# xiaozhah/Aligner

Measured on AMD Instinct MI355X. Metric: aligned utterances/sec + frames/sec, [B=64,T_text=200,T_mel=1000], higher is better.
Workload: dtype f32; 1 GPU; configs[1]: similarity (L2, C=80) + monotonic alignment search, [B=64,T_text=200,T_mel=1000] fp32 per GPU, dense fp32 path + int32 durations out; batch_per_gpu=64, t_text=200, t_mel=1000, c_att=80, launch=hipGraph, batches_in_flight=3, parallelism=batch-sharded x1

## Files before the change

aligner_amd/csrc/api.cpp:

```cpp
#include <cstdarg>
#include <cstdio>
#include <cstdlib>

#include <mutex>
#include <cstring>
#include <map>
#include <utility>

#include "common.h"

namespace aligner {

char *error_buffer() {
    static thread_local char buf[512] = {0};
    return buf;
}

unsigned long long *g_debug_stamps = nullptr;

static int env_flag(const char *name) { const char *e = getenv(name); return e && e[0] && e[0] != '0'; }
int g_opt_fwdsum_one_wave = env_flag("ALIGNER_FWDSUM_ONE_WAVE");
int g_opt_fwdsum_serial = env_flag("ALIGNER_FWDSUM_SERIAL");
int g_opt_fwdsum_no_grad_stager = 0;
int g_opt_softattn_exact = env_flag("ALIGNER_SOFTATTN_EXACT");
int g_opt_mobo_drop_segment = -1;
int g_opt_mobo_start_lag = 0;
int g_opt_mobo_lanes = 0;
int g_opt_mobo_bwd_general = 0;
int g_opt_softattn_no_pair = 0;
int g_opt_softattn_rt_drop_merge = 0;
int g_opt_softattn_strips = env_flag("ALIGNER_SOFTATTN_STRIPS");
int g_opt_softattn_split = 0;
int g_opt_conv_narrow_ft = 0;
int g_opt_conv_no_ring = 0;
int g_opt_conv_no_fuse = 0;
int g_opt_conv_split_always = env_flag("ALIGNER_CONV_SPLIT_ALWAYS");
int g_opt_maxpath_no_split_walk = 0;
int g_opt_maxpath_zero_blocks = 0;
int g_opt_maxpath_no_mask_verify = 0;
int g_opt_maxpath_no_optimistic_mask = 0;
int g_opt_mobo_full_chain = 0;
int g_opt_mobo_stamp_wave = 0;

hipError_t ensure_dynamic_lds(const void *kernel, size_t bytes) {
    if (bytes <= 64 * 1024) return hipSuccess;
    int dev = 0;
    hipError_t e = hipGetDevice(&dev);
    if (e != hipSuccess) return e;
    static std::mutex mu;
    static std::map<std::pair<int, const void *>, size_t> granted;
    std::lock_guard<std::mutex> lock(mu);
    const auto key = std::make_pair(dev, kernel);
    auto it = granted.find(key);
    if (it != granted.end() && it->second >= bytes) return hipSuccess;
    e = hipFuncSetAttribute(kernel, hipFuncAttributeMaxDynamicSharedMemorySize, (int)bytes);
    if (e == hipSuccess) granted[key] = bytes;
    return e;
}

int device_cu_count() {
    int dev = 0, v = 0;
    if (hipGetDevice(&dev) != hipSuccess) return 1;
    static std::mutex mu;
    static std::map<int, int> counts;
    std::lock_guard<std::mutex> lock(mu);
    auto it = counts.find(dev);
    if (it != counts.end()) return it->second;
    if (hipDeviceGetAttribute(&v, hipDeviceAttributeMultiprocessorCount, dev) != hipSuccess || v < 1) v = 1;
    counts[dev] = v;
    return v;
}

int device_lds_limit() {
    int dev = 0;
    if (hipGetDevice(&dev) != hipSuccess) return 64 * 1024;
    static std::mutex mu;
    static std::map<int, int> limits;
    std::lock_guard<std::mutex> lock(mu);
    auto it = limits.find(dev);
    if (it != limits.end()) return it->second;
    int lim = 64 * 1024, v = 0;
    hipDeviceProp_t prop;
    if (hipGetDeviceProperties(&prop, dev) == hipSuccess && std::strncmp(prop.gcnArchName, "gfx950", 6) == 0)
        lim = 160 * 1024;
    else if (hipDeviceGetAttribute(&v, hipDeviceAttributeMaxSharedMemoryPerBlock, dev) == hipSuccess && v > 0)
        lim = v;
    limits[dev] = lim;
    return lim;
}

int fail(int code, const char *fmt, ...) {
    va_list ap;
    va_start(ap, fmt);
    vsnprintf(error_buffer(), 512, fmt, ap);
    va_end(ap);
    return code;
}

}

extern "C" {

int aligner_abi_version(void) { return ALIGNER_ABI_VERSION; }

const char *aligner_last_error(void) { return aligner::error_buffer(); }

void aligner_debug_set_stamps(void *stamps_dev) {
    aligner::g_debug_stamps = static_cast<unsigned long long *>(stamps_dev);
}

int aligner_debug_set_option(const char *name, int value) {
    if (!name) return aligner::fail(ALIGNER_EINVAL, "null option name");
    if (std::strcmp(name, "fwdsum_one_wave") == 0) { aligner::g_opt_fwdsum_one_wave = value; return ALIGNER_OK; }
    if (std::strcmp(name, "fwdsum_no_grad_stager") == 0) { aligner::g_opt_fwdsum_no_grad_stager = value; return ALIGNER_OK; }
    if (std::strcmp(name, "fwdsum_serial") == 0) { aligner::g_opt_fwdsum_serial = value; return ALIGNER_OK; }
    if (std::strcmp(name, "softattn_exact") == 0) { aligner::g_opt_softattn_exact = value; return ALIGNER_OK; }
    if (std::strcmp(name, "mobo_start_lag") == 0) { aligner::g_opt_mobo_start_lag = value; return ALIGNER_OK; }
    if (std::strcmp(name, "mobo_lanes") == 0) { aligner::g_opt_mobo_lanes = value; return ALIGNER_OK; }
    if (std::strcmp(name, "mobo_stamp_wave") == 0) { aligner::g_opt_mobo_stamp_wave = value; return ALIGNER_OK; }
    if (std::strcmp(name, "mobo_full_chain") == 0) { aligner::g_opt_mobo_full_chain = value; return ALIGNER_OK; }
    if (std::strcmp(name, "softattn_split") == 0) { aligner::g_opt_softattn_split = value; return ALIGNER_OK; }
    if (std::strcmp(name, "conv_narrow_ft") == 0) { aligner::g_opt_conv_narrow_ft = value; return ALIGNER_OK; }
    if (std::strcmp(name, "conv_no_ring") == 0) { aligner::g_opt_conv_no_ring = value; return ALIGNER_OK; }
    if (std::strcmp(name, "conv_no_fuse") == 0) { aligner::g_opt_conv_no_fuse = value; return ALIGNER_OK; }
    if (std::strcmp(name, "conv_split_always") == 0) { aligner::g_opt_conv_split_always = value; return ALIGNER_OK; }
    if (std::strcmp(name, "maxpath_no_optimistic_mask") == 0) { aligner::g_opt_maxpath_no_optimistic_mask = value; return ALIGNER_OK; }
    if (std::strcmp(name, "maxpath_no_mask_verify") == 0) { aligner::g_opt_maxpath_no_mask_verify = value; return ALIGNER_OK; }
    if (std::strcmp(name, "maxpath_zero_blocks") == 0) { aligner::g_opt_maxpath_zero_blocks = value; return ALIGNER_OK; }
    if (std::strcmp(name, "maxpath_no_split_walk") == 0) { aligner::g_opt_maxpath_no_split_walk = value; return ALIGNER_OK; }
    if (std::strcmp(name, "softattn_strips") == 0) { aligner::g_opt_softattn_strips = value; return ALIGNER_OK; }
    if (std::strcmp(name, "softattn_rt_drop_merge") == 0) { aligner::g_opt_softattn_rt_drop_merge = value; return ALIGNER_OK; }
    if (std::strcmp(name, "softattn_no_pair") == 0) { aligner::g_opt_softattn_no_pair = value; return ALIGNER_OK; }
    if (std::strcmp(name, "mobo_bwd_general") == 0) { aligner::g_opt_mobo_bwd_general = value; return ALIGNER_OK; }
    if (std::strcmp(name, "mobo_drop_segment") == 0) { aligner::g_opt_mobo_drop_segment = value; return ALIGNER_OK; }
    return aligner::fail(ALIGNER_EINVAL, "unknown option '%s'", name);
}

int aligner_device_count(void) {
    int n = 0;
    if (hipGetDeviceCount(&n) != hipSuccess) {
        (void)hipGetLastError();
        return 0;
    }
    return n;
}

}
```

aligner_amd/csrc/common.h:

```cpp
#pragma once
#include <hip/hip_runtime.h>
#include <cstdarg>
#include <cstdio>

#include "aligner_amd.h"

namespace aligner {

char *error_buffer();
int   fail(int code, const char *fmt, ...) __attribute__((format(printf, 2, 3)));

#define ALIGNER_HIP_CHECK(expr)                                                        \
    do {                                                                               \
        hipError_t _e = (expr);                                                        \
        if (_e != hipSuccess)                                                          \
            return ::aligner::fail(ALIGNER_EHIP, "%s failed: %s (%s:%d)", #expr,       \
                                   hipGetErrorString(_e), __FILE__, __LINE__);         \
    } while (0)

inline int dtype_size(int dt) {
    switch (dt) {
        case ALIGNER_DT_F32: return 4;
        case ALIGNER_DT_F16: return 2;
        case ALIGNER_DT_BF16: return 2;
        case ALIGNER_DT_F64: return 8;
        case ALIGNER_DT_I32: return 4;
        case ALIGNER_DT_U8: return 1;
        case ALIGNER_DT_I64: return 8;
        default: return 0;
    }
}

hipError_t ensure_dynamic_lds(const void *kernel, size_t bytes);

int device_lds_limit();
int device_cu_count();

extern unsigned long long *g_debug_stamps;
extern int g_opt_softattn_exact;
extern int g_opt_mobo_start_lag;
extern int g_opt_mobo_stamp_wave;
extern int g_opt_mobo_full_chain;
extern int g_opt_conv_narrow_ft;
extern int g_opt_conv_no_ring;
extern int g_opt_maxpath_no_optimistic_mask;
extern int g_opt_maxpath_no_mask_verify;
extern int g_opt_maxpath_zero_blocks;
extern int g_opt_maxpath_no_split_walk;
extern int g_opt_conv_no_fuse;
extern int g_opt_conv_split_always;
extern int g_opt_softattn_split;
extern int g_opt_softattn_strips;
extern int g_opt_softattn_rt_drop_merge;
extern int g_opt_softattn_no_pair;
extern int g_opt_mobo_bwd_general;
extern int g_opt_mobo_lanes;
extern int g_opt_mobo_drop_segment;
extern int g_opt_fwdsum_no_grad_stager;
extern int g_opt_fwdsum_serial;
extern int g_opt_fwdsum_one_wave;

inline size_t align_up(size_t v, size_t a) { return (v + a - 1) / a * a; }

}
```

aligner_amd/csrc/mobo.hip:

```cpp
#include <hip/hip_runtime.h>

#include <cmath>
#include <cstdint>

#include "aligner_amd.h"
#include "common.h"

namespace aligner {

constexpr float MB_NEG = -1e30f;
constexpr float MB_DEADF = -1e7f;
constexpr int MB_DEADM = -(1 << 24);
constexpr unsigned MB_FILL = 0xFFFFFFFFu;
constexpr float MB_LOG2E = 1.4426950408889634f, MB_LN2 = 0.6931471805599453f;
constexpr int MB_SPIN_LIMIT = 1 << 21;

struct MoboParams {
    const void *e;
    const int *t_xs, *t_ys;
    float *log_alpha;
    int *boundaries;
    int *durations;
    float *map_score;
    float *Lw;
// ... 942 lines not shown
                const unsigned h_c = h_nx;
                issue_halo(i + 1 < I ? i + 1 : I - 1);
                const int bo = (i & 1) * W;
                auto halo_entry = [&](int h, unsigned x) {
                    if (x == MB_FILL) {
                        const unsigned *r = ring_in + (size_t)i * 3 * D + h;
                        int spins = 0;
                        do {
                            __builtin_amdgcn_s_sleep(2);
                            x = mb_ring_load(r);
                            if (++spins > p.spin_limit) gave_up = true;
                        } while (x == MB_FILL && !gave_up);
                    }
                    sV[bo + h] = (x == MB_FILL) ? MB_NEG : __builtin_bit_cast(float, x);
                };
                if (fetches) halo_entry(hl, h_c);
                if (D > 64) {
#pragma unroll 1
                    for (int h = hl + 64; h < D; h += 64) halo_entry(h, MB_FILL);
                }
                mb_lds_barrier();
            }
        }
        if (gave_up) {
            atomicOr(p.status, ALIGNER_ST_INTERNAL);
            p.failw[b] = 1;
        }
        return;
    }

    const int je = (j1 < 1 ? 1 : (j1 > J ? J : j1)) - 1;
    const int kl = j1 > J - 1 ? J - 1 : j1;
    unsigned e_n1, e_n2;
    float L_n1, L_n2;
    auto issue = [&](int i, unsigned &e_o, float &L_o) {
        const size_t ro = ubase + (size_t)i * p.Ty;
        e_o = mb_load_raw<VT>(p.e, ro + je);
        L_o = p.Lw[ro + kl];
    };
    issue(i0, e_n1, L_n1);
    mb_ring_store(trash, 0u);
    mb_ring_store(trash, 0u);
    issue(i0 + 1 < I ? i0 + 1 : I - 1, e_n2, L_n2);
    mb_ring_store(trash, 0u);
    mb_ring_store(trash, 0u);
    auto do_row = [&](const int i, unsigned &e_s, float &L_s) {
        int lo, hi;
        mb_bounds(I, J, D, i, lo, hi);
        const unsigned e_c = e_s;
        const float L_c = L_s;
        issue(i + 2 < I ? i + 2 : I - 1, e_s, L_s);
        const int bo = (i & 1) * W;
        {
            const float L = (j1 < J) ? L_c : MB_NEG;
            float v = (L > MB_DEADF && de > MB_DEADF) ? de - L : MB_NEG;
            v = (v > MB_DEADF) ? v : MB_NEG;
            *(mine ? sV + bo + D + pi : sSpare) = v;
            mb_ring_store(publishes ? ring_out + (size_t)i * 3 * D + (j1 - (bnd - D)) : trash, __builtin_bit_cast(unsigned, v));
        }
        mb_lds_barrier();
        {
            const float ev = mb_value<VT>(e_c) * MB_LOG2E;
            const bool feasible = mine && j1 >= lo && j1 <= hi;
            const float *vv = sV + bo + (mine ? pi : 0) + w0;
            const int cnt = w1 - w0;
            float best = MB_NEG;
            int qb = 0, c = 0;
            for (const int r8 = cnt & 7; c < r8; ++c) {
                const float v = vv[c];
                if (v >= best) { best = v; qb = c; }
            }
#define MB_MAX3F(a_, b_, c_) __builtin_fmaxf(__builtin_fmaxf(a_, b_), c_)
#define MB_MAX3I(a_, b_, c_) ((a_) > (b_) ? ((a_) > (c_) ? (a_) : (c_)) : ((b_) > (c_) ? (b_) : (c_)))
            if (((cnt - c) & 15) == 0) {
#pragma unroll 1
                for (; c < cnt; c += 16) {
                    float v[16];
#pragma unroll
                    for (int u = 0; u < 16; ++u) v[u] = vv[c + u];
                    const float m0 = MB_MAX3F(v[0], v[1], v[2]), m1 = MB_MAX3F(v[3], v[4], v[5]), m2 = MB_MAX3F(v[6], v[7], v[8]);
                    const float m3 = MB_MAX3F(v[9], v[10], v[11]), m4 = MB_MAX3F(v[12], v[13], v[14]);
                    const float vm = __builtin_fmaxf(MB_MAX3F(m0, m1, m2), MB_MAX3F(m3, m4, v[15]));
                    int q[16];
#pragma unroll
                    for (int u = 0; u < 16; ++u) q[u] = (v[u] == vm) ? u : -1;
                    const int q0 = MB_MAX3I(q[0], q[1], q[2]), q1 = MB_MAX3I(q[3], q[4], q[5]), q2 = MB_MAX3I(q[6], q[7], q[8]);
                    const int q3 = MB_MAX3I(q[9], q[10], q[11]), q4 = MB_MAX3I(q[12], q[13], q[14]);
                    const int qa = MB_MAX3I(q0, q1, q2), qc = MB_MAX3I(q3, q4, q[15]);
                    const int qi = qa > qc ? qa : qc;
                    const bool take = vm >= best;
                    best = take ? vm : best;
                    qb = take ? c + qi : qb;
                }
            } else {
#pragma unroll 1
                for (; c < cnt; c += 8) {
                    float v[8];
#pragma unroll
                    for (int u = 0; u < 8; ++u) v[u] = vv[c + u];
                    float vm = v[0];
#pragma unroll
                    for (int u = 1; u < 8; ++u) vm = __builtin_fmaxf(vm, v[u]);
                    int qi = 0;
#pragma unroll
                    for (int u = 1; u < 8; ++u) qi = (v[u] == vm) ? u : qi;
                    if (vm >= best) { best = vm; qb = c + qi; }
                }
            }
#undef MB_MAX3F
#undef MB_MAX3I
            qb += w0;
#pragma unroll
            for (int m = 1; m < H; m <<= 1) {
                const float bo_ = mb_quad_xor_f(best, m);
                const int qo = mb_quad_xor_i(qb, m);
                const bool take = bo_ > best || (bo_ == best && qo > qb);
                best = take ? bo_ : best;
                qb = take ? qo : qb;
            }
            float dev = MB_NEG;
            int dur = 0;
            if (feasible && ev > MB_DEADF && best > MB_DEADF) {
                dev = ev + best;
                dur = D - qb;
                if (!(dev > MB_DEADF)) { dev = MB_NEG; dur = 0; }
            }
            de = dev;
            unsigned short *bp = lead ? backb + (size_t)i * p.bstride + j1 : reinterpret_cast<unsigned short *>(trash);
            *bp = (unsigned short)dur;
        }
    };
#pragma unroll 1
    for (int i = i0; i <= i1; i += 2) {
        do_row(i, e_n1, L_n1);
        if (i + 1 > i1) break;
        do_row(i + 1, e_n2, L_n2);
    }
    if (lead && j1 == J && i1 == I - 1 && p.map_score)
        p.map_score[b] = (de > MB_DEADF) ? de * MB_LN2 : -__builtin_huge_valf();
    if (i1 + 1 < I) {
        const int i = i1 + 1;
        if (publishes) {
            const float Lr = p.Lw[ubase + (size_t)i * p.Ty + kl];
            const float L = (j1 < J) ? Lr : MB_NEG;
            float v = (L > MB_DEADF && de > MB_DEADF) ? de - L : MB_NEG;
            v = (v > MB_DEADF) ? v : MB_NEG;
            mb_ring_store(ring_out + (size_t)i * 3 * D + (j1 - (bnd - D)), __builtin_bit_cast(unsigned, v));
        }
        dead_rows(i1 + 2, I);
        if (lead && j1 == J && p.map_score) p.map_score[b] = -__builtin_huge_valf();
    }
}

template <int VT, int H>
__global__ __launch_bounds__(1024) void mobo_chain_sum_kernel(MoboParams p) {
    extern __shared__ __attribute__((aligned(16))) unsigned char smem[];
    const int tid = threadIdx.x;
    const bool has_helper = p.S > 1;
    const int T = (int)blockDim.x - (has_helper ? 64 : 0);
    const bool helper = tid >= T;
    const int b = blockIdx.x / p.S, sg = blockIdx.x - b * p.S;
    const int D = p.D;
    int I = p.t_xs[b], J = p.t_ys[b];
    I = I > p.Tx ? p.Tx : I;
    J = J > p.Ty ? p.Ty : J;
    const bool ok = I >= 1 && J >= I && (long long)J <= (long long)I * D;
    if (!ok) {
        if (sg == 0 && tid == 0) atomicOr(p.status, ALIGNER_ST_BAD_LENGTHS);
        return;
    }
    const int P = J + 1;
    int Sb = P / D;
    Sb = Sb < 1 ? 1 : (Sb > p.S ? p.S : Sb);
    const int n = (P + Sb - 1) / Sb;
    const int a = sg * n;
    if (sg >= Sb || a >= P) return;
    const int bnd = (a + n < P) ? a + n : P;
    const bool has_next = (sg + 1 < Sb) && (a + n < P) && sg != p.drop_seg;
    const int W = p.nmax + D;
    int *sM = reinterpret_cast<int *>(smem);
    float *sS = reinterpret_cast<float *>(sM + 2 * W);
    float *sT = sS + 2 * W;
    int *sRep = reinterpret_cast<int *>(sT + 2 * W);
    float *sSpare = reinterpret_cast<float *>(sRep + 64);
    if (tid < 32) { sRep[2 * tid] = MB_DEADM; sRep[2 * tid + 1] = 0; }
    for (int h = tid; h < D; h += T) {
        sM[h] = MB_DEADM;  sM[W + h] = MB_DEADM;
        sS[h] = 0.f;       sS[W + h] = 0.f;
        sT[h] = 0.f;       sT[W + h] = 0.f;
    }
    mb_lds_barrier();
    const int pi = tid / H, sub = tid - pi * H;
    const int j1 = a + pi;
    const bool mine = !helper && j1 < bnd;
    const bool lead = mine && sub == 0;
    float la = (j1 == 0) ? 0.f : MB_NEG;
    const size_t ubase = (size_t)b * p.Tx * p.Ty;
    unsigned *trash = p.trash + (size_t)blockIdx.x * 1024 + tid;
    unsigned *ring_out = p.ring + ((size_t)b * (p.S - 1) + (has_next ? sg : 0)) * (size_t)p.Tx * 3 * D;
    const unsigned *ring_in = p.ring + ((size_t)b * (p.S - 1) + (sg > 0 ? sg - 1 : 0)) * (size_t)p.Tx * 3 * D;
    const int hl = tid - T;
    const bool publishes = has_next && lead && j1 >= bnd - D;
    const int w0 = (sub * D) / H, w1 = ((sub + 1) * D) / H;
    const int wave = tid >> 6, lane = tid & 63;
    int i0, i1;
    mb_active_rows(I, J, D, a, bnd, i0, i1);
    auto dead_rows = [&](int from, int to) {
        for (int i = from; i < to; ++i) {
            if (has_next && !helper)
                for (int h = tid; h < D; h += T) {
                    unsigned *r = ring_out + (size_t)i * 3 * D + h;
                    mb_ring_store(r, __builtin_bit_cast(unsigned, (float)MB_DEADM));
                    mb_ring_store(r + D, 0u);
                }
            if (lead && j1 >= 1) p.log_alpha[ubase + (size_t)i * p.Ty + (j1 - 1)] = -__builtin_huge_valf();
        }
    };
    if (i1 < 0) {
        dead_rows(0, I);
        return;
    }
    dead_rows(0, i0);
    bool gave_up = false;
    int R = 0;

    if (helper) {
        if (sg > 0) {
            if (p.start_lag > 0) {
                int ig = i0 + p.start_lag;
                ig = ig > I - 1 ? I - 1 : ig;
                const unsigned *r = ring_in + (size_t)ig * 3 * D + (hl < D ? hl : 0) + D;
                int spins = 0;
                while (mb_ring_load(r) == MB_FILL && !gave_up) {
                    __builtin_amdgcn_s_sleep(8);
                    if (++spins > p.spin_limit) gave_up = true;
                }
            }
            const bool fetches = hl < D;
            unsigned h0_nx, h1_nx;
            auto issue_halo = [&](int i) {
                const unsigned *r = fetches ? ring_in + (size_t)i * 3 * D + hl : trash;
                h0_nx = mb_ring_load(r);
                h1_nx = mb_ring_load(r + (fetches ? D : 0));
            };
            issue_halo(i0);
#pragma unroll 1
            for (int i = i0; i <= i1; ++i) {
                const unsigned h_c0 = h0_nx, h_c1 = h1_nx;
                issue_halo(i + 1 < I ? i + 1 : I - 1);
                const int bo = (i & 1) * W;
                int Mstat = MB_DEADM;
                bool fits = true;
                auto halo_entry = [&](int h, unsigned x0, unsigned x1) {
                    if (x0 == MB_FILL || x1 == MB_FILL) {
                        const unsigned *r = ring_in + (size_t)i * 3 * D + h;
                        int spins = 0;
                        do {
                            __builtin_amdgcn_s_sleep(2);
                            x0 = mb_ring_load(r);
                            x1 = mb_ring_load(r + D);
                            if (++spins > p.spin_limit) gave_up = true;
                        } while ((x0 == MB_FILL || x1 == MB_FILL) && !gave_up);
                    }
                    const bool bad = (x0 == MB_FILL || x1 == MB_FILL);
                    const int M = bad ? MB_DEADM : (int)__builtin_bit_cast(float, x0);
                    const float sv = bad ? 0.f : __builtin_bit_cast(float, x1);
                    sM[bo + h] = M;
                    sS[bo + h] = sv;
                    sT[bo + h] = __builtin_ldexpf(sv, M - R);
                    if (M != MB_DEADM) {
                        Mstat = Mstat > M ? Mstat : M;
                        fits = fits && M >= R - 100 && M <= R + 100;
                    }
                };
                if (fetches) halo_entry(hl, h_c0, h_c1);
                if (D > 64) {
#pragma unroll 1
                    for (int h = hl + 64; h < D; h += 64) halo_entry(h, MB_FILL, MB_FILL);
                }
                {
                    const int wm = mb_wave_max_i32(Mstat);
                    const bool wfit = __builtin_amdgcn_ballot_w64(!fits) == 0;
                    mb_report_put(sRep, i & 1, wave, wm, wfit ? 0 : 1);
                }
                mb_lds_barrier();
                int Rn, slow_;
                mb_report_get(sRep, i & 1, lane, Rn, slow_);
                R = (Rn != MB_DEADM) ? Rn : R;
            }
        }
        if (gave_up) {
            atomicOr(p.status, ALIGNER_ST_INTERNAL);
            p.failw[b] = 1;
        }
        return;
    }

    const int je = (j1 < 1 ? 1 : (j1 > J ? J : j1)) - 1;
    const int kl = j1 > J - 1 ? J - 1 : j1;
    unsigned e_n1, e_n2;
    float L_n1, L_n2;
    auto issue = [&](int i, unsigned &e_o, float &L_o) {
        const size_t ro = ubase + (size_t)i * p.Ty;
        e_o = mb_load_raw<VT>(p.e, ro + je);
        L_o = p.Lw[ro + kl];
    };
// ... 328 lines not shown
    return pl.total;
}

int aligner_boundary_search_backward(const void *energies, int energy_dtype, const int32_t *t_xs, const int32_t *t_ys,
                                     int max_duration, const float *log_alpha, const float *grad_log_alpha,
                                     const float *grad_gamma, float *grad_energies_out, void *workspace,
                                     size_t workspace_bytes, int B, int Tx, int Ty, void *stream) {
    if (!energies || !t_xs || !t_ys || !log_alpha || !grad_energies_out || !workspace) return fail(ALIGNER_EINVAL, "null pointer");
    if (!grad_log_alpha && !grad_gamma) return fail(ALIGNER_EINVAL, "no cotangent: grad_log_alpha and grad_gamma are both null");
    if (B < 0 || Tx < 1 || Ty < 1) return fail(ALIGNER_EINVAL, "bad shape B=%d Tx=%d Ty=%d", B, Tx, Ty);
    if (max_duration < 1) return fail(ALIGNER_EINVAL, "max_duration %d < 1", max_duration);
    const int vt = energy_dtype == ALIGNER_DT_F32 ? 0 : energy_dtype == ALIGNER_DT_BF16 ? 1 : energy_dtype == ALIGNER_DT_F16 ? 2 : -1;
    if (vt < 0) return fail(ALIGNER_EINVAL, "energy dtype %d not supported (F32, BF16, F16)", energy_dtype);
    if (B == 0) return ALIGNER_OK;
    if (B > 65535 || Tx > 65535) return fail(ALIGNER_EDOM, "grid too large");
    if ((max_duration > Ty ? Ty : max_duration) > 65535) return fail(ALIGNER_EDOM, "max_duration %d too large", max_duration);
    MoboBwdPlan pl;
    const int prc = mobo_bwd_plan(B, Tx, Ty, max_duration, pl, false);
    if (prc) return prc;
    const MoboPlan &f = pl.f;
    if ((long long)B * f.S > 0x7fffffffLL) return fail(ALIGNER_EDOM, "grid too large");
    if (workspace_bytes < pl.total) return fail(ALIGNER_ENOSPC, "workspace %zu < %zu bytes", workspace_bytes, pl.total);
    unsigned char *ws = static_cast<unsigned char *>(workspace);
    hipStream_t s = static_cast<hipStream_t>(stream);
    const size_t nlds = (size_t)(MB_NCH + f.D + 4) * 12;
    if (nlds > (size_t)device_lds_limit()) return fail(ALIGNER_EDOM, "max_duration %d needs %zu bytes of LDS", f.D, nlds);
    {
        MoboParams p{};
        p.e = energies;  p.t_xs = t_xs;  p.t_ys = t_ys;
        p.Lw = reinterpret_cast<float *>(ws + pl.L_off);
        p.ring = reinterpret_cast<unsigned *>(ws + pl.ring_off);
        p.failw = reinterpret_cast<int *>(ws + pl.fail_off);
        p.status = reinterpret_cast<int *>(ws + pl.status_off);
        p.B = B;  p.Tx = Tx;  p.Ty = Ty;  p.D = f.D;  p.S = f.S;  p.nmax = f.nmax;
        const dim3 grid((Ty + MB_NCH - 1) / MB_NCH, Tx, B);
        auto launch = [&](auto kern) -> int {
            ALIGNER_HIP_CHECK(ensure_dynamic_lds(reinterpret_cast<const void *>(kern), nlds));
            hipLaunchKernelGGL(kern, grid, dim3(256), nlds, s, p, (unsigned long long)pl.ring_words);
            ALIGNER_HIP_CHECK(hipGetLastError());
            return ALIGNER_OK;
        };
        const int rc = vt == 0 ? launch(mobo_norm_kernel<0>) : vt == 1 ? launch(mobo_norm_kernel<1>) : launch(mobo_norm_kernel<2>);
        if (rc) return rc;
    }
    float *Gw = reinterpret_cast<float *>(ws + pl.G_off);
    MoboBwdParams q{energies, t_xs, t_ys, log_alpha, grad_log_alpha, grad_gamma, grad_energies_out,
                    reinterpret_cast<float *>(ws + pl.L_off), grad_gamma ? Gw : grad_log_alpha, Gw,
                    reinterpret_cast<float *>(ws + pl.Y_off), reinterpret_cast<unsigned *>(ws + pl.ring_off),
                    reinterpret_cast<int *>(ws + pl.fail_off), reinterpret_cast<unsigned *>(ws + pl.trash_off),
                    reinterpret_cast<int *>(ws + pl.status_off), B, Tx, Ty, f.D, f.S, f.nmax, g_opt_mobo_start_lag,
                    g_opt_mobo_drop_segment, g_opt_mobo_drop_segment >= 0 ? 2048 : MB_SPIN_LIMIT, g_debug_stamps, g_opt_mobo_stamp_wave};
    if (grad_gamma) {
        hipLaunchKernelGGL(mobo_bwd_cotangent_kernel, dim3(Tx, B), dim3(256), 0, s, q);
        ALIGNER_HIP_CHECK(hipGetLastError());
    }
    {
        auto launch = [&](auto kern) -> int {
            ALIGNER_HIP_CHECK(ensure_dynamic_lds(reinterpret_cast<const void *>(kern), pl.lds));
            hipLaunchKernelGGL(kern, dim3((unsigned)B * f.S), dim3(pl.T), pl.lds, s, q);
            ALIGNER_HIP_CHECK(hipGetLastError());
            return ALIGNER_OK;
        };
#define MB_BWD_LAUNCH(VT_)                                                                                             \
    (pl.multi ? launch(mobo_bwd_chain_kernel<VT_, true>)                                                              \
     : g_opt_mobo_bwd_general ? launch(mobo_bwd_chain_kernel<VT_, false>)                                             \
     : g_debug_stamps ? MB_BWD_LAUNCH_H(VT_, true) : MB_BWD_LAUNCH_H(VT_, false))
#define MB_BWD_LAUNCH_H(VT_, ST_)                                                                                     \
    (f.H == 1 ? launch(mobo_bwd_chain_one_kernel<VT_, 1, ST_>) : f.H == 2 ? launch(mobo_bwd_chain_one_kernel<VT_, 2, ST_>) \
                                                                           : launch(mobo_bwd_chain_one_kernel<VT_, 4, ST_>))
        if (g_opt_mobo_bwd_general && !pl.multi) pl.T = (f.nmax + 63) / 64 * 64;
        const int rc = vt == 0 ? MB_BWD_LAUNCH(0) : vt == 1 ? MB_BWD_LAUNCH(1) : MB_BWD_LAUNCH(2);
#undef MB_BWD_LAUNCH
#undef MB_BWD_LAUNCH_H
        if (rc) return rc;
    }
    {
        const dim3 grid((Ty + MB_NCH - 1) / MB_NCH, Tx, B);
        auto launch = [&](auto kern) -> int {
            ALIGNER_HIP_CHECK(ensure_dynamic_lds(reinterpret_cast<const void *>(kern), nlds));
            hipLaunchKernelGGL(kern, grid, dim3(256), nlds, s, q);
            ALIGNER_HIP_CHECK(hipGetLastError());
            return ALIGNER_OK;
        };
        const int rc = vt == 0 ? launch(mobo_bwd_grad_kernel<0>) : vt == 1 ? launch(mobo_bwd_grad_kernel<1>) : launch(mobo_bwd_grad_kernel<2>);
        if (rc) return rc;
    }
    return ALIGNER_OK;
}

size_t aligner_boundary_search_workspace_bytes_ex(int B, int Tx, int Ty, int max_duration) {
    if (B < 0 || Tx < 1 || Ty < 1 || max_duration < 1) return 0;
    MoboPlan pl;
    if (mobo_plan(B, Tx, Ty, max_duration, pl, true) != ALIGNER_OK) return 0;
    return pl.total;
}

size_t aligner_boundary_search_workspace_bytes(int B, int Tx, int Ty) {
    if (B < 0 || Tx < 1 || Ty < 1) return 0;
    const size_t fixed = 256 + align_up((size_t)B * sizeof(int), 256) + align_up((size_t)B * Tx * Ty * sizeof(float), 256) +
                         align_up(((size_t)(B > 1024 ? B : 1024 + B) * 1024 + 64) * sizeof(unsigned), 256) +
                         align_up((size_t)B * Tx * ((size_t)Ty + 8) * sizeof(unsigned short), 256);
    return fixed + align_up((size_t)B * Tx * 3 * ((size_t)Ty + 1) * sizeof(unsigned), 256) + 256;
}

int aligner_boundary_search(const void *energies, int energy_dtype, const int32_t *t_xs, const int32_t *t_ys,
                            int max_duration, int32_t *boundaries_out, int32_t *durations_out, float *map_score_out,
                            float *log_alpha_out, float *gamma_out, void *workspace, size_t workspace_bytes, int B,
                            int Tx, int Ty, void *stream) {
    if (!energies || !t_xs || !t_ys || !workspace) return fail(ALIGNER_EINVAL, "null pointer");
    if (!boundaries_out && !log_alpha_out) return fail(ALIGNER_EINVAL, "nothing asked for: boundaries_out and log_alpha_out are both null");
    if (!boundaries_out && (durations_out || map_score_out))
        return fail(ALIGNER_EINVAL, "durations / map_score need boundaries_out (the MAP sequence is searched or it is not)");
    if (B < 0 || Tx < 1 || Ty < 1) return fail(ALIGNER_EINVAL, "bad shape B=%d Tx=%d Ty=%d", B, Tx, Ty);
    if (max_duration < 1) return fail(ALIGNER_EINVAL, "max_duration %d < 1", max_duration);
    const int vt = energy_dtype == ALIGNER_DT_F32 ? 0 : energy_dtype == ALIGNER_DT_BF16 ? 1 : energy_dtype == ALIGNER_DT_F16 ? 2 : -1;
    if (vt < 0) return fail(ALIGNER_EINVAL, "energy dtype %d not supported (F32, BF16, F16)", energy_dtype);
    if (gamma_out && !log_alpha_out) return fail(ALIGNER_EINVAL, "gamma needs the log_alpha buffer as well");
    if (B == 0) return ALIGNER_OK;
    if (B > 65535 || Tx > 65535) return fail(ALIGNER_EDOM, "grid too large");
    if ((max_duration > Ty ? Ty : max_duration) > 65535) return fail(ALIGNER_EDOM, "max_duration %d too large", max_duration);
    MoboPlan pl;
    const int prc = mobo_plan(B, Tx, Ty, max_duration, pl, false);
    if (prc) return prc;
    if ((long long)B * pl.S > 0x7fffffffLL) return fail(ALIGNER_EDOM, "grid too large");
    if (workspace_bytes < pl.total) return fail(ALIGNER_ENOSPC, "workspace %zu < %zu bytes", workspace_bytes, pl.total);
    unsigned char *ws = static_cast<unsigned char *>(workspace);
    hipStream_t s = static_cast<hipStream_t>(stream);
    MoboParams p{energies, t_xs, t_ys, log_alpha_out, boundaries_out, durations_out, map_score_out,
                 reinterpret_cast<float *>(ws + pl.L_off), reinterpret_cast<unsigned short *>(ws + pl.back_off),
                 reinterpret_cast<unsigned *>(ws + pl.ring_off), reinterpret_cast<int *>(ws + pl.fail_off),
                 reinterpret_cast<unsigned *>(ws + pl.trash_off),
                 reinterpret_cast<int *>(ws + pl.status_off), B, Tx, Ty, pl.D, pl.S, pl.nmax, pl.bstride, g_opt_mobo_start_lag, g_debug_stamps,
                 g_opt_mobo_drop_segment, g_opt_mobo_drop_segment >= 0 ? 2048 : MB_SPIN_LIMIT};
    {
        const size_t nlds = (size_t)(MB_NCH + pl.D + 4) * 12;
        if (nlds > (size_t)device_lds_limit()) return fail(ALIGNER_EDOM, "max_duration %d needs %zu bytes of LDS", pl.D, nlds);
        const dim3 grid((Ty + MB_NCH - 1) / MB_NCH, Tx, B);
        auto launch = [&](auto kern) -> int {
            ALIGNER_HIP_CHECK(ensure_dynamic_lds(reinterpret_cast<const void *>(kern), nlds));
            hipLaunchKernelGGL(kern, grid, dim3(256), nlds, s, p, (unsigned long long)pl.ring_words);
            ALIGNER_HIP_CHECK(hipGetLastError());
            return ALIGNER_OK;
        };
        const int rc = vt == 0 ? launch(mobo_norm_kernel<0>) : vt == 1 ? launch(mobo_norm_kernel<1>) : launch(mobo_norm_kernel<2>);
        if (rc) return rc;
    }
    {
        auto launch = [&](auto kern) -> int {
            ALIGNER_HIP_CHECK(ensure_dynamic_lds(reinterpret_cast<const void *>(kern), pl.lds));
            hipLaunchKernelGGL(kern, dim3((unsigned)B * pl.S), dim3(pl.T), pl.lds, s, p);
            ALIGNER_HIP_CHECK(hipGetLastError());
            return ALIGNER_OK;
        };
        int rc;
#define MB_LAUNCH_NP(VT_)                                                                               \
    (pl.NP != 1 ? launch(mobo_chain_kernel<VT_, true>)                                                  \
     : (!boundaries_out && !g_opt_mobo_full_chain && !g_debug_stamps) ? MB_LAUNCH_SUM(VT_)              \
     : log_alpha_out ? MB_LAUNCH_H(VT_, true)                                                           \
     : (g_opt_mobo_full_chain || g_debug_stamps) ? MB_LAUNCH_H(VT_, false) : MB_LAUNCH_MAP(VT_))
#define MB_LAUNCH_SUM(VT_)                                                                              \
    (pl.H == 1 ? launch(mobo_chain_sum_kernel<VT_, 1>) : pl.H == 2 ? launch(mobo_chain_sum_kernel<VT_, 2>) \
                                                                    : launch(mobo_chain_sum_kernel<VT_, 4>))
#define MB_LAUNCH_MAP(VT_)                                                                              \
    (pl.H == 1 ? launch(mobo_chain_map_kernel<VT_, 1>) : pl.H == 2 ? launch(mobo_chain_map_kernel<VT_, 2>) \
                                                                    : launch(mobo_chain_map_kernel<VT_, 4>))
#define MB_LAUNCH_H(VT_, LA_)                                                                            \
    (g_debug_stamps ? MB_LAUNCH_ST(VT_, LA_, true) : MB_LAUNCH_ST(VT_, LA_, false))
#define MB_LAUNCH_ST(VT_, LA_, ST_)                                                                      \
    (pl.H == 1 ? launch(mobo_chain_one_kernel<VT_, LA_, 1, ST_>) : pl.H == 2 ? launch(mobo_chain_one_kernel<VT_, LA_, 2, ST_>) \
                                                                              : launch(mobo_chain_one_kernel<VT_, LA_, 4, ST_>))
        rc = vt == 0 ? MB_LAUNCH_NP(0) : vt == 1 ? MB_LAUNCH_NP(1) : MB_LAUNCH_NP(2);
        if (rc) return rc;
    }
    if (boundaries_out) {
        ALIGNER_HIP_CHECK(ensure_dynamic_lds(reinterpret_cast<const void *>(mobo_backtrack_kernel), pl.bt_lds));
        hipLaunchKernelGGL(mobo_backtrack_kernel, dim3(B), dim3(256), pl.bt_lds, s, p, pl.RB);
        ALIGNER_HIP_CHECK(hipGetLastError());
    }
    if (gamma_out) {
        hipLaunchKernelGGL(mobo_gamma_kernel, dim3(Tx, B), dim3(256), 0, s, log_alpha_out, t_xs, t_ys, gamma_out, Tx, Ty);
        ALIGNER_HIP_CHECK(hipGetLastError());
    }
    return ALIGNER_OK;
}

}
```

Baseline: 2.152 million utterances/s.

## Add DPP suffix/prefix-max scan kernel for MAP monotonic alignment chain

Adds a new chain kernel for the MAP (boundaries) path that replaces the per-cell loop over the duration window with a segmented max scan. Floats are mapped to order-preserving integer keys and reduced with DPP row suffix/prefix operations; per-row partial maxima are combined through LDS. The window max and argmax then cost a handful of lane operations instead of D sequential compares. It is gated on D being 16, 32 or 64 and adds a helper wave for halo exchange between segments, which brings more code complexity and new tie-breaking logic to keep correct.

```diff
diff --git a/aligner_amd/csrc/api.cpp b/aligner_amd/csrc/api.cpp
--- a/aligner_amd/csrc/api.cpp
+++ b/aligner_amd/csrc/api.cpp
@@ -40,6 +40,7 @@
 int g_opt_maxpath_no_mask_verify = 0;
 int g_opt_maxpath_no_optimistic_mask = 0;
 int g_opt_mobo_full_chain = 0;
+int g_opt_mobo_map_window_loop = 0;
 int g_opt_mobo_stamp_wave = 0;
 
 hipError_t ensure_dynamic_lds(const void *kernel, size_t bytes) {
@@ -119,6 +120,7 @@
     if (std::strcmp(name, "mobo_lanes") == 0) { aligner::g_opt_mobo_lanes = value; return ALIGNER_OK; }
     if (std::strcmp(name, "mobo_stamp_wave") == 0) { aligner::g_opt_mobo_stamp_wave = value; return ALIGNER_OK; }
     if (std::strcmp(name, "mobo_full_chain") == 0) { aligner::g_opt_mobo_full_chain = value; return ALIGNER_OK; }
+    if (std::strcmp(name, "mobo_map_window_loop") == 0) { aligner::g_opt_mobo_map_window_loop = value; return ALIGNER_OK; }
     if (std::strcmp(name, "softattn_split") == 0) { aligner::g_opt_softattn_split = value; return ALIGNER_OK; }
     if (std::strcmp(name, "conv_narrow_ft") == 0) { aligner::g_opt_conv_narrow_ft = value; return ALIGNER_OK; }
     if (std::strcmp(name, "conv_no_ring") == 0) { aligner::g_opt_conv_no_ring = value; return ALIGNER_OK; }
diff --git a/aligner_amd/csrc/common.h b/aligner_amd/csrc/common.h
--- a/aligner_amd/csrc/common.h
+++ b/aligner_amd/csrc/common.h
@@ -41,6 +41,7 @@
 extern int g_opt_mobo_start_lag;
 extern int g_opt_mobo_stamp_wave;
 extern int g_opt_mobo_full_chain;
+extern int g_opt_mobo_map_window_loop;
 extern int g_opt_conv_narrow_ft;
 extern int g_opt_conv_no_ring;
 extern int g_opt_maxpath_no_optimistic_mask;
diff --git a/aligner_amd/csrc/mobo.hip b/aligner_amd/csrc/mobo.hip
--- a/aligner_amd/csrc/mobo.hip
+++ b/aligner_amd/csrc/mobo.hip
@@ -1118,6 +1118,248 @@
     }
 }
 
+typedef int mb_i2 __attribute__((ext_vector_type(2)));
+
+__device__ __forceinline__ int mb_key(float v) {
+    const int b = __builtin_bit_cast(int, v);
+    return b ^ ((b >> 31) & 0x7fffffff);
+}
+__device__ __forceinline__ float mb_unkey(int k) { return __builtin_bit_cast(float, k ^ ((k >> 31) & 0x7fffffff)); }
+constexpr int MB_NEG_KEY = (int)(0xf149f2cau ^ 0x7fffffffu);
+
+#define MB_DPP_MAX_I(x_, ctrl_)                                                                                          \
+    {                                                                                                                    \
+        const int o_ = __builtin_amdgcn_update_dpp((int)0x80000000, x_, ctrl_, 0xF, 0xF, false);                         \
+        x_ = x_ > o_ ? x_ : o_;                                                                                          \
+    }
+#define MB_DPP_MIN_I(x_, ctrl_)                                                                                          \
+    {                                                                                                                    \
+        const int o_ = __builtin_amdgcn_update_dpp(0x7fffffff, x_, ctrl_, 0xF, 0xF, false);                              \
+        x_ = x_ < o_ ? x_ : o_;                                                                                          \
+    }
+__device__ __forceinline__ void mb_row_suffix(int k, int g, int &S, int &q) {
+    S = k;
+    MB_DPP_MAX_I(S, 0x101)
+    MB_DPP_MAX_I(S, 0x102)
+    MB_DPP_MAX_I(S, 0x104)
+    MB_DPP_MAX_I(S, 0x108)
+    const int y = __builtin_amdgcn_update_dpp(MB_NEG_KEY, S, 0x101, 0xF, 0xF, false);
+    q = k > y ? g : 0x7fffffff;
+    MB_DPP_MIN_I(q, 0x101)
+    MB_DPP_MIN_I(q, 0x102)
+    MB_DPP_MIN_I(q, 0x104)
+    MB_DPP_MIN_I(q, 0x108)
+}
+__device__ __forceinline__ void mb_row_prefix(int k, int g, int &P, int &q) {
+    const int x = __builtin_amdgcn_update_dpp(MB_NEG_KEY, k, 0x111, 0xF, 0xF, false);
+    P = x;
+    MB_DPP_MAX_I(P, 0x111)
+    MB_DPP_MAX_I(P, 0x112)
+    MB_DPP_MAX_I(P, 0x114)
+    MB_DPP_MAX_I(P, 0x118)
+    q = x == P ? g - 1 : (int)0x80000000;
+    MB_DPP_MAX_I(q, 0x111)
+    MB_DPP_MAX_I(q, 0x112)
+    MB_DPP_MAX_I(q, 0x114)
+    MB_DPP_MAX_I(q, 0x118)
+}
+#undef MB_DPP_MAX_I
+#undef MB_DPP_MIN_I
+
+template <int VT, int DD>
+__global__ __launch_bounds__(1024) void mobo_chain_map_scan_kernel(MoboParams p) {
+    extern __shared__ __attribute__((aligned(16))) unsigned char smem[];
+    static_assert(DD == 16 || DD == 32 || DD == 64, "whole DPP rows, at most one wave of halo");
+    static_assert(__builtin_bit_cast(unsigned, MB_NEG) == 0xf149f2cau, "MB_NEG_KEY is the image of MB_NEG");
+    const int tid = threadIdx.x;
+    const bool has_helper = p.S > 1;
+    const int T = (int)blockDim.x - (has_helper ? 64 : 0);
+    const bool helper = tid >= T;
+    const int b = blockIdx.x / p.S, sg = blockIdx.x - b * p.S;
+    constexpr int D = DD;
+    int I = p.t_xs[b], J = p.t_ys[b];
+    I = I > p.Tx ? p.Tx : I;
+    J = J > p.Ty ? p.Ty : J;
+    const bool ok = I >= 1 && J >= I && (long long)J <= (long long)I * D;
+    if (!ok) {
+        if (sg == 0 && tid == 0) atomicOr(p.status, ALIGNER_ST_BAD_LENGTHS);
+        return;
+    }
+    const int P = J + 1;
+    int Sb = P / D;
+    Sb = Sb < 1 ? 1 : (Sb > p.S ? p.S : Sb);
+    const int n = (P + Sb - 1) / Sb;
+    const int a = sg * n;
+    if (sg >= Sb || a >= P) return;
+    const int bnd = (a + n < P) ? a + n : P;
+    const bool has_next = (sg + 1 < Sb) && (a + n < P) && sg != p.drop_seg;
+    const int W = D + T;
+    mb_i2 *sfx = reinterpret_cast<mb_i2 *>(smem);
+    for (int h = tid; h < D; h += T) {
+        sfx[h] = mb_i2{MB_NEG_KEY, 0};
+        sfx[W + h] = mb_i2{MB_NEG_KEY, 0};
+    }
+    mb_lds_barrier();
+    const int pi = tid;
+    const int j1 = a + pi;
+    const int g = D + pi;
+    const bool mine = !helper && j1 < bnd;
+    float de = (j1 == 0) ? 0.f : MB_NEG;
+    const size_t ubase = (size_t)b * p.Tx * p.Ty;
+    unsigned short *backb = p.back + (size_t)b * p.Tx * p.bstride;
+    unsigned *trash = p.trash + (size_t)blockIdx.x * 1024 + tid;
+    unsigned *ring_out = p.ring + ((size_t)b * (p.S - 1) + (has_next ? sg : 0)) * (size_t)p.Tx * 3 * D + 2 * D;
+    const unsigned *ring_in = p.ring + ((size_t)b * (p.S - 1) + (sg > 0 ? sg - 1 : 0)) * (size_t)p.Tx * 3 * D + 2 * D;
+    const int hl = tid - T;
+    const bool publishes = has_next && mine && j1 >= bnd - D;
+    int i0, i1;
+    mb_active_rows(I, J, D, a, bnd, i0, i1);
+    auto dead_rows = [&](int from, int to) {
+        if (has_next && !helper)
+            for (int i = from; i < to; ++i)
+                for (int h = tid; h < D; h += T) mb_ring_store(ring_out + (size_t)i * 3 * D + h, __builtin_bit_cast(unsigned, MB_NEG));
+    };
+    if (i1 < 0) {
+        dead_rows(0, I);
+        if (mine && j1 == J && p.map_score) p.map_score[b] = -__builtin_huge_valf();
+        return;
+    }
+    dead_rows(0, i0);
+    bool gave_up = false;
+
+    if (helper) {
+        if (sg > 0) {
+            if (p.start_lag > 0) {
+                int ig = i0 + p.start_lag;
+                ig = ig > I - 1 ? I - 1 : ig;
+                const unsigned *r = ring_in + (size_t)ig * 3 * D + (hl < D ? hl : 0);
+                int spins = 0;
+                while (mb_ring_load(r) == MB_FILL && !gave_up) {
+                    __builtin_amdgcn_s_sleep(8);
+                    if (++spins > p.spin_limit) gave_up = true;
+                }
+            }
+            const bool fetches = hl < D;
+            unsigned h_nx;
+            auto issue_halo = [&](int i) { h_nx = mb_ring_load(fetches ? ring_in + (size_t)i * 3 * D + hl : trash); };
+            issue_halo(i0);
+#pragma unroll 1
+            for (int i = i0; i <= i1; ++i) {
+                unsigned x = h_nx;
+                issue_halo(i + 1 < I ? i + 1 : I - 1);
+                if (fetches && x == MB_FILL) {
+                    const unsigned *r = ring_in + (size_t)i * 3 * D + hl;
+                    int spins = 0;
+                    do {
+                        __builtin_amdgcn_s_sleep(2);
+                        x = mb_ring_load(r);
+                        if (++spins > p.spin_limit) gave_up = true;
+                    } while (x == MB_FILL && !gave_up);
+                }
+                const float hv = (!fetches || x == MB_FILL) ? MB_NEG : __builtin_bit_cast(float, x);
+                int Sk, Sq;
+                mb_row_suffix(mb_key(hv), hl, Sk, Sq);
+                if (fetches) sfx[(i & 1) * W + hl] = mb_i2{Sk, Sq};
+                mb_lds_barrier();
+            }
+        }
+        if (gave_up) {
+            atomicOr(p.status, ALIGNER_ST_INTERNAL);
+            p.failw[b] = 1;
+        }
+        return;
+    }
+
+    const int je = (j1 < 1 ? 1 : (j1 > J ? J : j1)) - 1;
+    const int kl = j1 > J - 1 ? J - 1 : j1;
+    unsigned e_n1, e_n2;
+    float L_n1, L_n2;
+    auto issue = [&](int i, unsigned &e_o, float &L_o) {
+        const size_t ro = ubase + (size_t)i * p.Ty;
+        e_o = mb_load_raw<VT>(p.e, ro + je);
+        L_o = p.Lw[ro + kl];
+    };
+    issue(i0, e_n1, L_n1);
+    mb_ring_store(trash, 0u);
+    mb_ring_store(trash, 0u);
+    issue(i0 + 1 < I ? i0 + 1 : I - 1, e_n2, L_n2);
+    mb_ring_store(trash, 0u);
+    mb_ring_store(trash, 0u);
+    const int row0 = (g & ~15) - D;
+    auto do_row = [&](const int i, unsigned &e_s, float &L_s) {
+        int lo, hi;
+        mb_bounds(I, J, D, i, lo, hi);
+        const unsigned e_c = e_s;
+        const float L_c = L_s;
+        issue(i + 2 < I ? i + 2 : I - 1, e_s, L_s);
+        const int bo = (i & 1) * W;
+        int Pk, Pq;
+        {
+            const float L = (j1 < J) ? L_c : MB_NEG;
+            float v = (L > MB_DEADF && de > MB_DEADF) ? de - L : MB_NEG;
+            v = (v > MB_DEADF) ? v : MB_NEG;
+            mb_ring_store(publishes ? ring_out + (size_t)i * 3 * D + (j1 - (bnd - D)) : trash, __builtin_bit_cast(unsigned, v));
+            const int k = mb_key(v);
+            int Sk, Sq;
+            mb_row_suffix(k, g, Sk, Sq);
+            sfx[bo + g] = mb_i2{Sk, Sq};
+            mb_row_prefix(k, g, Pk, Pq);
+        }
+        asm volatile("s_waitcnt lgkmcnt(0)\n\ts_barrier" : "+v"(Pk), "+v"(Pq) : : "memory");
+        {
+            const float ev = mb_value<VT>(e_c) * MB_LOG2E;
+            const bool feasible = mine && j1 >= lo && j1 <= hi;
+            mb_i2 pc[D / 16];
+            pc[0] = sfx[bo + g - D];
+#pragma unroll
+            for (int r = 1; r < D / 16; ++r) pc[r] = sfx[bo + row0 + 16 * r];
+            int kb = pc[0].x, gb = pc[0].y;
+#pragma unroll
+            for (int r = 1; r < D / 16; ++r) {
+                const bool take = pc[r].x >= kb;
+                kb = take ? pc[r].x : kb;
+                gb = take ? pc[r].y : gb;
+            }
+            {
+                const bool take = Pk >= kb;
+                kb = take ? Pk : kb;
+                gb = take ? Pq : gb;
+            }
+            const float best = mb_unkey(kb);
+            float dev = MB_NEG;
+            int dur = 0;
+            if (feasible && ev > MB_DEADF && best > MB_DEADF) {
+                dev = ev + best;
+                dur = g - gb;
+                if (!(dev > MB_DEADF)) { dev = MB_NEG; dur = 0; }
+            }
+            de = dev;
+            unsigned short *bp = mine ? backb + (size_t)i * p.bstride + j1 : reinterpret_cast<unsigned short *>(trash);
+            *bp = (unsigned short)dur;
+        }
+    };
+#pragma unroll 1
+    for (int i = i0; i <= i1; i += 2) {
+        do_row(i, e_n1, L_n1);
+        if (i + 1 > i1) break;
+        do_row(i + 1, e_n2, L_n2);
+    }
+    if (mine && j1 == J && i1 == I - 1 && p.map_score)
+        p.map_score[b] = (de > MB_DEADF) ? de * MB_LN2 : -__builtin_huge_valf();
+    if (i1 + 1 < I) {
+        const int i = i1 + 1;
+        if (publishes) {
+            const float Lr = p.Lw[ubase + (size_t)i * p.Ty + kl];
+            const float L = (j1 < J) ? Lr : MB_NEG;
+            float v = (L > MB_DEADF && de > MB_DEADF) ? de - L : MB_NEG;
+            v = (v > MB_DEADF) ? v : MB_NEG;
+            mb_ring_store(ring_out + (size_t)i * 3 * D + (j1 - (bnd - D)), __builtin_bit_cast(unsigned, v));
+        }
+        dead_rows(i1 + 2, I);
+        if (mine && j1 == J && p.map_score) p.map_score[b] = -__builtin_huge_valf();
+    }
+}
+
 template <int VT, int H>
 __global__ __launch_bounds__(1024) void mobo_chain_sum_kernel(MoboParams p) {
     extern __shared__ __attribute__((aligned(16))) unsigned char smem[];
@@ -1752,7 +1994,20 @@
             ALIGNER_HIP_CHECK(hipGetLastError());
             return ALIGNER_OK;
         };
+        const bool scan_form = boundaries_out && !log_alpha_out && pl.NP == 1 && (pl.D == 16 || pl.D == 32 || pl.D == 64) &&
+                               !g_opt_mobo_full_chain && !g_debug_stamps && !g_opt_mobo_map_window_loop;
+        const int scan_T = (pl.nmax + 63) / 64 * 64;
+        auto launch_scan = [&](auto kern) -> int {
+            const size_t lds = (size_t)2 * 8 * (pl.D + scan_T);
+            ALIGNER_HIP_CHECK(ensure_dynamic_lds(reinterpret_cast<const void *>(kern), lds));
+            hipLaunchKernelGGL(kern, dim3((unsigned)B * pl.S), dim3(scan_T + (pl.S > 1 ? 64 : 0)), lds, s, p);
+            ALIGNER_HIP_CHECK(hipGetLastError());
+            return ALIGNER_OK;
+        };
         int rc;
+#define MB_LAUNCH_SCAN(VT_)                                                                              \
+    (pl.D == 16 ? launch_scan(mobo_chain_map_scan_kernel<VT_, 16>) : pl.D == 32 ? launch_scan(mobo_chain_map_scan_kernel<VT_, 32>) \
+                                                                                : launch_scan(mobo_chain_map_scan_kernel<VT_, 64>))
 #define MB_LAUNCH_NP(VT_)                                                                               \
     (pl.NP != 1 ? launch(mobo_chain_kernel<VT_, true>)                                                  \
      : (!boundaries_out && !g_opt_mobo_full_chain && !g_debug_stamps) ? MB_LAUNCH_SUM(VT_)              \
@@ -1769,7 +2024,8 @@
 #define MB_LAUNCH_ST(VT_, LA_, ST_)                                                                      \
     (pl.H == 1 ? launch(mobo_chain_one_kernel<VT_, LA_, 1, ST_>) : pl.H == 2 ? launch(mobo_chain_one_kernel<VT_, LA_, 2, ST_>) \
                                                                               : launch(mobo_chain_one_kernel<VT_, LA_, 4, ST_>))
-        rc = vt == 0 ? MB_LAUNCH_NP(0) : vt == 1 ? MB_LAUNCH_NP(1) : MB_LAUNCH_NP(2);
+        if (scan_form) rc = vt == 0 ? MB_LAUNCH_SCAN(0) : vt == 1 ? MB_LAUNCH_SCAN(1) : MB_LAUNCH_SCAN(2);
+        else rc = vt == 0 ? MB_LAUNCH_NP(0) : vt == 1 ? MB_LAUNCH_NP(1) : MB_LAUNCH_NP(2);
         if (rc) return rc;
     }
     if (boundaries_out) {
```

Measured after the change: 2.102 million utterances/s. 0.977x the previous value.
